# amathislab/BUCTD

Measured on AMD Instinct MI355X. Metric: images/sec (train) BUCTD-CoAM-W48 384x288, higher is better.
Workload: dtype f32 (3x3 convs: operands split exactly into 3 bf16 pieces, 6 bf16 MFMAs per product, fp32 accumulate - fp32-class); 1 GPU; BUCTD-CoAM-W48 (pose_hrnet_coam, ATT_MODULES [F,T,F,F], colored condition) 384x288 CrowdPose-14kpt full train step: fwd + JointsMSE + bwd + grad all-reduce + Adam + arg-max accuracy decode; global_batch=32, batch_per_gpu=32, input=N x 6 x 384 x 288 fp32, params=115581770, parallelism=dp1, hip_streams=4, conv_math=bf16x6, step_graph=False

## Files before the change

buctd_amd/_C.py:

```python
import ctypes as C
import os

import torch

_HERE = os.path.dirname(os.path.abspath(__file__))
LIB_PATH = os.path.join(_HERE, "lib", "libbuctd_hip.so")


class ConvDesc(C.Structure):
    _fields_ = [(n, C.c_int) for n in ("N", "H", "W", "Ci", "Co", "R", "S", "stride", "pad", "Ho", "Wo")]


class BasicBlockDesc(C.Structure):
    _fields_ = ([(n, C.c_int) for n in ("N", "H", "W", "C")] +
                [(n, C.c_void_p) for n in ("x", "w1_fwd", "w2_fwd", "w1_bwd", "w2_bwd", "gamma1", "beta1", "gamma2", "beta2",
                                           "running_mean1", "running_var1", "running_mean2", "running_var2")] +
                [(n, C.c_float) for n in ("eps1", "momentum1", "eps2", "momentum2")] +
                [(n, C.c_void_p) for n in ("z1", "z2", "y", "acc", "stat")])


class BasicBlockGrads(C.Structure):
    _fields_ = ([(n, C.c_void_p) for n in ("dy", "dz2", "dres", "dy1", "dz1", "dx", "dw1", "dw2", "dgamma1", "dbeta1",
                                           "dgamma2", "dbeta2")] +
                [(n, C.c_int) for n in ("acc_w1", "acc_w2", "acc_bn1", "acc_bn2")] +
# ... 208 lines not shown
    "buctd_gconv_x6_prep_item": (_I, [_I, _I, _I, _P, _I, _P, _P]),
    "buctd_gconv_x6_prep_batched": (_I, [_P, _I, _P]),
    "buctd_gconv_x6_stats_groups": (_I, [_I] * 6 + [_PI, _PI]),
    "buctd_gconv_x6_fwd": (_I, [_I] * 6 + [_P] * 6 + [_I, _P, _P, _P, _P]),
    "buctd_gconv_x6_dgrad": (_I, [_I] * 6 + [_P] * 4 + [_P]),
    "buctd_mha_fwd_bf16x6_workspace": (_SZ, [_I, _I, _I]),
    "buctd_mha_fwd_bf16x6_ws": (_I, [_I, _I, _I, _P, _P, _P, _I, _I, _F, _P, _P, _P, _SZ, _P]),
    "buctd_mha_train_supported": (_I, [_I, _I]),
    "buctd_mha_fwd_train": (_I, [_I, _I, _I, _P, _P, _P, _I, _I, _F, _F, _U64, _P, _P, _P]),
    "buctd_mha_bwd_workspace": (_SZ, [_I, _I]),
    "buctd_mha_bwd": (_I, [_I, _I, _I, _P, _P, _P, _I, _I, _P, _P, _P, _F, _F, _U64, _P, _P, _I, _P, _I, _P, _SZ, _P]),
    "buctd_mha_fwd_train_dseed": (_I, [_I, _I, _I, _P, _P, _P, _I, _I, _F, _F, _P, _P, _P, _P]),
    "buctd_mha_bwd_dseed": (_I, [_I, _I, _I, _P, _P, _P, _I, _I, _P, _P, _P, _F, _F, _P, _P, _P, _I, _P, _I, _P, _SZ, _P]),
    "buctd_mha_heads_fwd_supported": (_I, [_I, _I, _I]),
    "buctd_mha_heads_fwd": (_I, [C.POINTER(MhaArgs), _P]),
    "buctd_mha_heads_fwd_bf16x6": (_I, [C.POINTER(MhaArgs), _P]),
    "buctd_mha_heads_train_supported": (_I, [_I, _I, _I]),
    "buctd_mha_heads_fwd_train": (_I, [C.POINTER(MhaArgs), _U64, _P]),
    "buctd_mha_heads_bwd_workspace": (_SZ, [_I, _I, _I]),
    "buctd_mha_heads_bwd": (_I, [C.POINTER(MhaArgs), _U64, _P, _SZ, _P]),
    "buctd_mha_heads_fwd_train_dseed": (_I, [C.POINTER(MhaArgs), _P, _P]),
    "buctd_mha_heads_bwd_dseed": (_I, [C.POINTER(MhaArgs), _P, _P, _SZ, _P]),
    "buctd_nms_workspace": (_SZ, [_I]),
    "buctd_nms": (_I, [_P, _P, _P, _I, _I, _F, _P, _SZ, _P]),
    "buctd_cpu_nms": (_I, [_P, _I, _P, _F, _P, _P]),
    "buctd_argmax_decode_refined": (_I, [_P, _I, _I, _I, _P, _P, _P, _P, _P]),
    "buctd_argmax_decode_dark": (_I, [_P, _I, _I, _I, _P, _P, _P, _P, _P]),
    "buctd_gaussian_target": (_I, [_P, _P, _I, _I, _I, _I, _F, _F, _F, _P, _P, _P]),
    "buctd_cond_render_workspace": (_SZ, [_I, _I, _I, _I]),
    "buctd_cond_render": (_I, [_P, _I, _P, _I, _I, _I, _I, _I, _I, _P, _P, _SZ, _P]),
    "buctd_flipback_avg": (_I, [_P, _P, _P, _I, _I, _I, _I, _I, _P, _P]),
    "buctd_sgd_step": (_I, [_P, _P, _P, _L, _F, _F, _F, _I, _I, _F, _P]),
    "buctd_adam_step": (_I, [_P, _P, _P, _P, _L, _F, _F, _F, _F, _I, _F, _P]),
    "buctd_bf16_pack_conv": (_I, [_P, _L, _L, _L, _L, _I, _I, _I, _P, _P, _P, _P, _P, _F, _P, _P, _P]),
    "buctd_bf16_conv": (_I, [_P, _I, _I, _I, _I, _P, _P, _I, _I, _I, _I, _P, _I, _I, _P, _P, _SZ, _P]),
    "buctd_bf16_fuse_sum": (_I, [C.POINTER(_P), _PI, _I, _I, _I, _I, _I, _I, _P, _P]),
    "buctd_bf16_from_f32": (_I, [_P, _L, _P, _P]),
}

_lib = None


class BuctdHipError(RuntimeError):
    pass


def lib():
    global _lib
    if _lib is None:
        if not os.path.isfile(LIB_PATH):
            raise BuctdHipError(
                f"{LIB_PATH} is missing - build it with `make` (or __graft_entry__.build()); "
                "buctd_amd has no CPU / eager fallback")
        handle = C.CDLL(LIB_PATH, mode=C.RTLD_GLOBAL)
        for name, (res, args) in SIGNATURES.items():
            fn = getattr(handle, name)
            fn.restype = res
            fn.argtypes = args
        _lib = handle
    return _lib


def check(rc, what=""):
    if rc != 0:
        msg = lib().buctd_last_error()
        raise BuctdHipError(f"{what} failed ({rc}): {msg.decode() if msg else ''}")
# ... 23 lines not shown
```

buctd_amd/csrc/conv_gather_x6.hip:

```cpp
#include "c3_lean.h"
#include <string.h>

#define GC_MAXT 9
#define GC_TAB_OFF (56 * 1024)

struct GcClass {
  int ntaps, nhs, nsteps;
  int oy0, ox0;
  long wp_off;
  unsigned pdy, pdx;
};

struct GcArgs {
  C3Args e;
  const float* src;
  const unsigned char* wp;
  int SH, SWd, SC, ss, cpt;
  int ncls;
  GcClass cls[4];
};

template <int MF, int NF, int WM, int WN, int MODE>
__global__ __launch_bounds__(256, 2) void gconv_x6_kernel(GcArgs p) {
  constexpr int BM = WM * MF * 16, BN = WN * NF * 16, ROWB = 96, PST = 32, BROW = 192;
  constexpr int QA = BM / 64;
  static_assert(WM * WN == 4 && BM % 64 == 0, "four waves, BM a multiple of 64");
  extern __shared__ __attribute__((aligned(16))) unsigned char smem[];
  const int t = threadIdx.x, lane = t & 63, wave = t >> 6;
  const int i16 = lane & 15, g = lane >> 4;
  const int wave_m = wave % WM, wave_n = wave / WM;
  const int bx = blockIdx.x, by = blockIdx.y;
  const GcClass& c = p.cls[blockIdx.z];
  C3Args e = p.e;
  e.oy0 = c.oy0; e.ox0 = c.ox0;
  const int p0 = bx * BM, n0 = by * BN;

// ... 94 lines not shown
      }
#undef GC_MMA
      if (mf < 2 * QA && mf < MF) {
        const int h = mf / QA, q = mf % QA;
        split_store_pk<3, PST>(smem + (size_t)(1 - SET) * ABUF + ((size_t)h * BM + arow + RSTEP * q) * ROWB, c4 * 4,
                               areg[1 - SET][h][q]);
      }
      __builtin_amdgcn_sched_barrier(0);
    }
    if (2 * QA > MF) {
#pragma unroll
      for (int i = MF; i < 2 * QA; ++i) {
        const int h = i / QA, q = i % QA;
        split_store_pk<3, PST>(smem + (size_t)(1 - SET) * ABUF + ((size_t)h * BM + arow + RSTEP * q) * ROWB, c4 * 4,
                               areg[1 - SET][h][q]);
      }
    }
    if (!PRIV) __syncthreads();
  };

  load_a(0, areg[0]);
  load_b(0, bnx[0]);
  load_a(1, areg[1]);
  store_a(areg[0], 0);
  if (!PRIV) __syncthreads();
  for (int st = 0; st < c.nsteps; st += 2) {
    step(st, IC<0>{});
    if (st + 1 < c.nsteps) step(st + 1, IC<1>{});
  }
  __syncthreads();
  if constexpr (MODE < 0) c3_epilogue<MF, NF, WM, WN>(e, acc, smem, bx, by, p0, n0);
  else c3l_epilogue<MF, NF, WM, WN, MODE>(e, acc, smem, reinterpret_cast<float*>(smem + GC_TAB_OFF), p0, n0);
}

struct GcPrep {
  const float* w;
  unsigned char* out;
  int Co, Ci, R, S, dir;
  int ncls;
  int ntaps[4], nsteps[4];
  long off[4];
  int tr[4][GC_MAXT], ts[4][GC_MAXT];
  long items[4];
};

__device__ __forceinline__ void gc_prep_body(const GcPrep& p) {
  const int nrows = p.dir ? p.Ci : p.Co, kc = p.dir ? p.Co : p.Ci, cpt = kc / 16;
  const long total = p.items[p.ncls - 1];
  for (long idx = (long)blockIdx.x * 256 + threadIdx.x; idx < total; idx += (long)gridDim.x * 256) {
    int cl = 0;
    while (idx >= p.items[cl]) ++cl;
    const long li = idx - (cl ? p.items[cl - 1] : 0);
    const int ks = (int)(li & 31);
    const long sr = li >> 5;
    const int row = (int)(sr % nrows), st = (int)(sr / nrows);
    const int hs = 2 * st + (ks >> 4);
    float v = 0.f;
    if (hs < p.ntaps[cl] * cpt) {
      const int tp = hs / cpt, k = (hs - tp * cpt) * 16 + (ks & 15);
      const int r = p.tr[cl][tp], s = p.ts[cl][tp];
      const int co = p.dir ? k : row, ci = p.dir ? row : k;
      v = p.w[(((long)co * p.R + r) * p.S + s) * p.Ci + ci];
    }
    unsigned char* o = p.out + p.off[cl] + ((size_t)st * nrows + row) * 192 + ks * 2;
#pragma unroll
    for (int q = 0; q < 3; ++q) {
      const __bf16 h = (__bf16)v;
      *reinterpret_cast<unsigned short*>(o + q * 64) = __builtin_bit_cast(unsigned short, h);
      v -= (float)h;
    }
  }
}

__global__ __launch_bounds__(256) void gconv_x6_prep_kernel(GcPrep p) { gc_prep_body(p); }

__global__ __launch_bounds__(256) void gconv_x6_prep_batched_kernel(const GcPrep* __restrict__ items) {
  gc_prep_body(items[blockIdx.y]);
// ... 417 lines not shown
```

buctd_amd/csrc/loss_decode.hip:

```cpp
#include "common.h"
#include "../../include/buctd_hip.h"

__global__ __launch_bounds__(256) void mse_partial_kernel(const float* __restrict__ pred, const float* __restrict__ gt,
                                                          const float* __restrict__ w, int HW, float gcoef,
                                                          float* __restrict__ part, float* __restrict__ grad) {
  __shared__ float sm[4];
  const long row = blockIdx.x;
  const float wt = w ? w[row] : 1.f;
  const float w2 = wt * wt;
  float s = 0.f;
  for (int i = threadIdx.x; i < HW; i += 256) {
    const float d = pred[row * HW + i] - gt[row * HW + i];
    s += d * d;
    if (grad) grad[row * HW + i] = gcoef * w2 * d;
  }
  s = block_sum_256(s, sm);
  if (threadIdx.x == 0) part[row] = s * w2;
}
__global__ __launch_bounds__(256) void mse_final_kernel(const float* __restrict__ part, int n, float coef,
                                                        float* __restrict__ loss) {
  __shared__ float sm[4];
  double s = 0.0;
  for (int i = threadIdx.x; i < n; i += 256) s += (double)part[i];
  float f = block_sum_256((float)s, sm);
  if (threadIdx.x == 0) loss[0] = f * coef;
}
extern "C" int buctd_joints_mse(const float* pred, const float* gt, const float* w, int N, int K, int HW, float* loss,
                                float* grad, float gscale, void* workspace, size_t workspace_bytes, void* stream) {
  BUCTD_CHECK_ARG(pred && gt && loss && N > 0 && K > 0 && HW > 0, "buctd_joints_mse: bad argument");
  const size_t need = (size_t)N * K * sizeof(float);
  if (!workspace || workspace_bytes < need) {
    buctd_set_error("buctd_joints_mse: workspace %zu bytes < required %zu", workspace_bytes, need);
    return BUCTD_EWORKSPACE;
// ... 494 lines not shown

__global__ __launch_bounds__(256) void flipback_avg_kernel(const float* __restrict__ a, const float* __restrict__ b,
                                                           const int32_t* __restrict__ perm, int K, int H, int W,
                                                           int shift, long total, float* __restrict__ out) {
  const long step = (long)gridDim.x * 256;
  for (long i = (long)blockIdx.x * 256 + threadIdx.x; i < total; i += step) {
    const int x = (int)(i % W);
    long r = i / W;
    const int y = (int)(r % H);
    r /= H;
    const int k = (int)(r % K);
    const long n = r / K;
    const int xs = (shift && x >= 1) ? x - 1 : x;
    const float fv = b[((n * K + perm[k]) * H + y) * W + (W - 1 - xs)];
    out[i] = (a[i] + fv) * 0.5f;
  }
}
extern "C" int buctd_flipback_avg(const float* a, const float* b, const int32_t* perm, int N, int K, int H, int W,
                                  int shift, float* out, void* stream) {
  BUCTD_CHECK_ARG(a && b && perm && out && N > 0 && K > 0 && H > 0 && W > 0, "buctd_flipback_avg: bad argument");
  const long total = (long)N * K * H * W;
  long blocks = (total + 255) / 256;
  if (blocks > 4096) blocks = 4096;
  hipLaunchKernelGGL(flipback_avg_kernel, dim3((unsigned)blocks), dim3(256), 0, (hipStream_t)stream, a, b, perm, K, H,
                     W, shift, total, out);
  BUCTD_CHECK_LAUNCH("buctd_flipback_avg");
  return BUCTD_OK;
}

__global__ __launch_bounds__(256) void adam_kernel(float* __restrict__ p, const float* __restrict__ g,
                                                   float* __restrict__ m, float* __restrict__ v, long n, float lr,
                                                   float b1, float b2, float eps, float bc1, float bc2_sqrt,
                                                   float gscale) {
  const float step_size = lr / bc1;
  const long n4 = n >> 2;
  const long step = (long)gridDim.x * 256;
  for (long i = (long)blockIdx.x * 256 + threadIdx.x; i < n4; i += step) {
    f32x4 pp = reinterpret_cast<f32x4*>(p)[i];
    const f32x4 gg = reinterpret_cast<const f32x4*>(g)[i] * gscale;
    f32x4 mm = reinterpret_cast<f32x4*>(m)[i];
    f32x4 vv = reinterpret_cast<f32x4*>(v)[i];
#pragma unroll
    for (int j = 0; j < 4; ++j) {
      mm[j] = b1 * mm[j] + (1.f - b1) * gg[j];
      vv[j] = b2 * vv[j] + (1.f - b2) * gg[j] * gg[j];
      const float denom = sqrtf(vv[j]) / bc2_sqrt + eps;
      pp[j] -= step_size * (mm[j] / denom);
    }
    reinterpret_cast<f32x4*>(p)[i] = pp;
    reinterpret_cast<f32x4*>(m)[i] = mm;
    reinterpret_cast<f32x4*>(v)[i] = vv;
  }
  for (long i = n4 * 4 + (long)blockIdx.x * 256 + threadIdx.x; i < n; i += step) {
    const float gg = g[i] * gscale;
    const float mm = b1 * m[i] + (1.f - b1) * gg;
    const float vv = b2 * v[i] + (1.f - b2) * gg * gg;
    m[i] = mm;
    v[i] = vv;
    p[i] -= step_size * (mm / (sqrtf(vv) / bc2_sqrt + eps));
  }
}
extern "C" int buctd_adam_step(float* p, const float* g, float* m, float* v, long n, float lr, float beta1,
                               float beta2, float eps, int step, float gscale, void* stream) {
  BUCTD_CHECK_ARG(p && g && m && v && n > 0 && step >= 1, "buctd_adam_step: bad argument");
  const double bc1 = 1.0 - pow((double)beta1, (double)step);
  const double bc2 = 1.0 - pow((double)beta2, (double)step);
  long blocks = ((n + 3) / 4 + 255) / 256;
  if (blocks > 4096) blocks = 4096;
  hipLaunchKernelGGL(adam_kernel, dim3((unsigned)blocks), dim3(256), 0, (hipStream_t)stream, p, g, m, v, n, lr, beta1,
                     beta2, eps, (float)bc1, (float)sqrt(bc2), gscale);
  BUCTD_CHECK_LAUNCH("buctd_adam_step");
  return BUCTD_OK;
}

__global__ __launch_bounds__(256) void sgd_kernel(float* __restrict__ p, const float* __restrict__ g, float* __restrict__ buf,
                                                  long n, float lr, float mu, float wd, int nesterov, int first, float gscale) {
  const long step = (long)gridDim.x * 256;
  for (long i = (long)blockIdx.x * 256 + threadIdx.x; i < n; i += step) {
    float pp = p[i];
    float gg = g[i] * gscale + wd * pp;
    if (mu != 0.f) {
      const float b = first ? gg : mu * buf[i] + gg;
      buf[i] = b;
      gg = nesterov ? gg + mu * b : b;
    }
    p[i] = pp - lr * gg;
  }
}
extern "C" int buctd_sgd_step(float* p, const float* g, float* momentum_buf, long n, float lr, float momentum,
                              float weight_decay, int nesterov, int first_step, float gscale, void* stream) {
  BUCTD_CHECK_ARG(p && g && n > 0 && (momentum == 0.f || momentum_buf), "buctd_sgd_step: bad argument");
  long blocks = (n + 255) / 256;
// ... 7 lines not shown
```

buctd_amd/engine.py:

```python
import os
import time

import torch
import torch.distributed as dist

from . import nn as bnn
from . import ops

_ALIGN = 4


class FlatParams:

    def __init__(self, module):
        bnn.prepare_module(module)
        self.params = []
        seen = set()
        for p in module.parameters():
            if id(p) not in seen:
                seen.add(id(p))
                self.params.append(p)
        if not self.params:
            raise ValueError("module has no parameters")
        dev = self.params[0].device
        self.offsets = {}
        off = 0
        for p in self.params:
            if p.dtype != torch.float32 or p.device != dev:
                raise ValueError("all parameters must be fp32 on one device")
            self.offsets[id(p)] = off
            off += (p.numel() + _ALIGN - 1) // _ALIGN * _ALIGN
        self.numel = off
        self.flat = torch.zeros(off, dtype=torch.float32, device=dev)
        self.grad = torch.zeros(off, dtype=torch.float32, device=dev)
        self._gviews = {}
        for p in self.params:
            v = self._view(self.flat, p)
            v.copy_(p.data)
            p.data = v
            self._gviews[id(p)] = self._view(self.grad, p)
        self.ready_cb = None
        ops.set_grad_arena(self)

    def _view(self, buf, p):
        o = self.offsets[id(p)]
        return torch.as_strided(buf, p.shape, p.stride(), o)

    def span(self, p):
        o = self.offsets[id(p)]
        return o, o + p.numel()

    def __call__(self, p):
        return self._gviews.get(id(p))

    def owns(self, p):
        return id(p) in self._gviews

    def grad_is_arena(self, p):
        return p.grad is not None and p.grad.data_ptr() == self._gviews[id(p)].data_ptr()

    def collect(self):
        for p in self.params:
            g = self._gviews[id(p)]
            if p.grad is None:
                if p.requires_grad:
                    g.zero_()
            elif not self.grad_is_arena(p):
                g.copy_(p.grad)
                p.grad = g

    def grad_runs(self):
        runs = []
        for p in self.params:
            if p.grad is None:
                continue
            s = self.offsets[id(p)]
            e = s + (p.numel() + _ALIGN - 1) // _ALIGN * _ALIGN
            if runs and runs[-1][1] == s:
                runs[-1][1] = e
            else:
                runs.append([s, e])
        return [(s, e) for s, e in runs]


class FusedAdam(torch.optim.Optimizer):

    def __init__(self, flat, lr=1e-3, betas=(0.9, 0.999), eps=1e-8, grad_sync=None):
        if not isinstance(flat, FlatParams):
            raise TypeError("FusedAdam works on an engine.FlatParams arena")
        super().__init__(flat.params, dict(lr=lr, betas=betas, eps=eps))
        self.flat = flat
        self.exp_avg = torch.zeros_like(flat.flat)
        self.exp_avg_sq = torch.zeros_like(flat.flat)
        self.step_count = 0
        self.grad_sync = grad_sync

    @torch.no_grad()
    def step(self, closure=None):
        if closure is not None:
            raise NotImplementedError("closures are not used on the BUCTD path")
        self.flat.collect()
        gscale = self.grad_sync() if self.grad_sync is not None else 1.0
        self.step_count += 1
        g = self.param_groups[0]
        ops.adam_step(self.flat.flat, self.flat.grad, self.exp_avg, self.exp_avg_sq, g["lr"], g["betas"][0],
                      g["betas"][1], g["eps"], self.step_count, gscale)
        ops.weights_updated()
        ops.refresh_prepared(self.flat.flat.device)
        if self.flat.flat.is_cuda:
            ops.acc_pool.reset(self.flat.flat.device)

    def zero_grad(self, set_to_none=True):
        self.zeroed = getattr(self, "zeroed", 0) + 1
        for p in self.flat.params:
            p.grad = None

    def state_dict(self):
        state = {}
        if self.step_count > 0:
            for i, p in enumerate(self.flat.params):
                o, e = self.flat.span(p)
                state[i] = {"step": torch.tensor(float(self.step_count)),
                            "exp_avg": torch.as_strided(self.exp_avg, p.shape, p.stride(), o).clone(),
                            "exp_avg_sq": torch.as_strided(self.exp_avg_sq, p.shape, p.stride(), o).clone()}
        groups = []
        for g in self.param_groups:
            d = {k: v for k, v in g.items() if k != "params"}
            for k, v in (("weight_decay", 0), ("amsgrad", False), ("maximize", False)):
                d.setdefault(k, v)
            d["params"] = list(range(len(self.flat.params)))
            groups.append(d)
        return {"state": state, "param_groups": groups}

    def load_state_dict(self, sd):
        if "state" not in sd:
            self.step_count = int(sd["step"])
            self.exp_avg.copy_(sd["exp_avg"])
            self.exp_avg_sq.copy_(sd["exp_avg_sq"])
        else:
            state = sd["state"]
# ... 648 lines not shown
```

buctd_amd/ops.py:

```python
import ctypes as C
import math

import torch

from . import _C
from ._C import ConvDesc, MatmulDesc, check, lib, ptr, stream_ptr

_capture = {"on": False, "events": set(), "allow_seeds": False, "seed_table": None, "seed_draws": 0}
_SEED_TABLE_SLOTS = 1024


def capturing():
    return _capture["on"]


def _new_event(stream=None):
    ev = torch.cuda.Event()
    ev.record(stream) if stream is not None else ev.record()
    if _capture["on"]:
        _capture["events"].add(id(ev))
        _capture.setdefault("keep", []).append(ev)
    return ev


# ... 413 lines not shown
    if _conv_math["mode"] != "bf16x6":
        return False
    items, live = [], []
    for ref in _gprep_registry["weights"]:
        w = ref()
        if w is None or not w.is_cuda or w.device != device:
            continue
        cache = getattr(w, "_buctd_gprep", None)
        if cache is None or cache[0][0] != w.data_ptr():
            continue
        live.append(ref)
        if cache[0] == (w.data_ptr(), w._version, epoch):
            continue
        Co, Ci = _wshape(w)[0], _wshape(w)[1]
        for direction in (0, 1):
            img = cache[2 + direction]
            if img is not None:
                items.append((cache[1], Ci, Co, w.data_ptr(), direction, img.data_ptr()))
        cache[0] = (w.data_ptr(), w._version, epoch)
    _gprep_registry["weights"] = live
    if not items:
        return False
    key = tuple(items)
    if _gprep_registry["table_key"] != key:
        isz = int(lib().buctd_gconv_x6_prep_item_bytes())
        buf = C.create_string_buffer(isz * len(items))
        base = C.addressof(buf)
        for i, (kind, Ci, Co, wptr, direction, iptr) in enumerate(items):
            check(lib().buctd_gconv_x6_prep_item(kind, Ci, Co, C.c_void_p(wptr), direction, C.c_void_p(iptr),
                                                 C.c_void_p(base + i * isz)), "gconv_x6_prep_item")
        _gprep_registry["table"] = torch.frombuffer(bytearray(buf.raw), dtype=torch.uint8).to(device)
        _gprep_registry["table_key"] = key
    check(lib().buctd_gconv_x6_prep_batched(ptr(_gprep_registry["table"]), len(items), stream_ptr()), "gconv_x6_prep_batched")
    return True


def _conv3x3_prepared(w, flip):
    import weakref
    Co, Ci = _wshape(w)[0], _wshape(w)[1]
    epoch = _weights_epoch["n"]
    key = (w.data_ptr(), w._version, epoch, _conv_math["mode"])
    cache = getattr(w, "_buctd_prep", None)
    if cache is not None and cache[0] != key and cache[0][:2] == key[:2] and cache[0][3:] == key[3:]:
        _prep_all(w.device)
    if cache is None or cache[0] != key:
        first = cache is None
        cache = [key, None, None]
        try:
            w._buctd_prep = cache
            if first:
                _prep_registry["weights"].append(weakref.ref(w))
        except (AttributeError, RuntimeError, TypeError):
            pass
    if cache[1 + flip] is None:
        nbytes = _c3fn("_prep_bytes")(Ci, Co, flip)
        img = torch.empty(nbytes, dtype=torch.uint8, device=w.device)
        check(_c3fn("_prep")(Ci, Co, ptr(w), flip, ptr(img), stream_ptr()), "conv3x3 prep")
        cache[1 + flip] = img
    _prep_wait(w.device)
    return cache[1 + flip]


def _conv3x3_bf16x3(x, w, flip, cin, cout, bias, scale, shift, residual, relu, stats, in_bn=None):
    N, H, W = x.shape[0], x.shape[1], x.shape[2]
    wp = _conv3x3_prepared(w, flip)
    y = torch.empty((N, H, W, cout), dtype=torch.float32, device=x.device)
# ... 429 lines not shown
           Kc=None, gsa=0, gsbk=0, Nc=None, gsbn=0, gsc=0, alpha=1.0, bias=None, bias_axis=0,
           a_off=0, b_off=0, c_off=0):
    d = MatmulDesc(batch, M, N, K, a_layout, b_layout, lda, ldb, ldc, stride_a, stride_b, stride_c,
                   K if Kc is None else Kc, gsa, gsbk, N if Nc is None else Nc, gsbn, gsc, alpha, bias_axis)
    need = lib().buctd_matmul_workspace(C.byref(d))
    ws = workspace(need, A.device) if need else None
    pa = C.c_void_p(A.data_ptr() + 4 * a_off)
    pb = C.c_void_p(B.data_ptr() + 4 * b_off)
    pc = C.c_void_p(Cout.data_ptr() + 4 * c_off)
    check(lib().buctd_matmul(C.byref(d), pa, pb, ptr(bias), pc, ptr(ws), ws.numel() if ws is not None else 0,
                             stream_ptr()), "matmul")
    return Cout


def x6_image(src, V, K, role, *, vs, ks, vg=0, vgs=0, kg=0, kgs=0, off=0, out=None):
    need = lib().buctd_x6_image_bytes(V, K, role)
    if out is None or out.numel() < need:
        out = torch.empty(need, dtype=torch.uint8, device=src.device)
    check(lib().buctd_x6_image(C.c_void_p(src.data_ptr() + 4 * off), V, K, vg, vgs, vs, kg, kgs, ks, role, ptr(out),
                               stream_ptr()), "x6_image")
    return out


def x6_gemm(a_image, b_image, Cout, M, N, K, *, ldc, Nc=0, gsc=0, bias=None, bias_axis=0, alpha=1.0, c_off=0):
    check(lib().buctd_x6_gemm(M, N, K, ptr(a_image), ptr(b_image), ptr(bias), bias_axis, alpha,
                              C.c_void_p(Cout.data_ptr() + 4 * c_off), ldc, Nc, gsc, stream_ptr()), "x6_gemm")
    return Cout


def _x6_weight_image(w, V, K, transposed):
    key = (w.data_ptr(), w._version, _weights_epoch["n"])
    cache = getattr(w, "_buctd_x6img", None)
    if cache is None or cache["key"] != key:
        cache = {"key": key}
        try:
            w._buctd_x6img = cache
        except (AttributeError, RuntimeError, TypeError):
            pass
    tag = "t" if transposed else "n"
    if tag not in cache:
        ld = w.shape[1]
        cache[tag] = x6_image(w, V, K, 0, vs=1, ks=ld) if transposed else x6_image(w, V, K, 0, vs=ld, ks=1)
        cache[tag + "_ev"] = _new_event()
        cache[tag + "_stream"] = torch.cuda.current_stream(w.device).cuda_stream
    elif torch.cuda.current_stream(w.device).cuda_stream != cache[tag + "_stream"]:
        _wait_event(torch.cuda.current_stream(w.device), cache[tag + "_ev"])
    return cache[tag]


def fc_o_x6_ok(T, rows):
    return _conv_math["mode"] == "bf16x6" and T >= 512 and rows >= 192


def bn_finalize(part, info, rows, Cn, eps, momentum, running_mean, running_var):
    mean = torch.empty(Cn, dtype=torch.float32, device=part.device)
    invstd = torch.empty(Cn, dtype=torch.float32, device=part.device)
    counts = info[2] if len(info) > 2 else None
    check(lib().buctd_bn_finalize(ptr(part), ptr(counts), info[0], info[1], rows, Cn, eps, momentum, ptr(mean), ptr(invstd),
                                  ptr(running_mean), ptr(running_var), stream_ptr()), "bn_finalize")
    return mean, invstd


class BnAccInput:

    def __init__(self, acc, rows, bn, training=True, relu=True):
        Cn = acc.Cn
        dev = bn.weight.device
        self.acc, self.rows, self.gamma, self.beta, self.relu = acc, int(rows), bn.weight, bn.bias, relu
        self.eps = bn.eps
        self.momentum = 0.1 if bn.momentum is None else bn.momentum
        stat = torch.empty((2, Cn), dtype=torch.float32, device=dev)
        self.mean, self.invstd = stat[0], stat[1]
        track = bn.track_running_stats and training
        self.rm = bn.running_mean if track else None
        self.rv = bn.running_var if track else None
# ... 1369 lines not shown
```

include/buctd_hip.h:

```cpp
#ifndef BUCTD_HIP_H
#define BUCTD_HIP_H
#include <stddef.h>
#include <stdint.h>

#ifdef __cplusplus
extern "C" {
#endif

int buctd_version(void);
const char* buctd_last_error(void);

typedef struct {
  int N, H, W, Ci;
  int Co, R, S;
  int stride, pad;
  int Ho, Wo;
} buctd_conv_desc;

int buctd_conv2d_fwd_thin(const buctd_conv_desc* d);
int buctd_conv2d_fwd(const buctd_conv_desc* d, const float* x, const float* w, const float* bias,
                     const float* scale, const float* shift, const float* residual, int relu, float* y,
                     float* stats_partials, void* stream);
int buctd_conv2d_dgrad(const buctd_conv_desc* d, const float* dy, const float* w, const float* bias, float* dx,
                       float* stats_partials, void* stream);
// ... 277 lines not shown
  float eps1, momentum1, eps2, momentum2;
  float *z1, *z2, *y;
  void* acc;
  float* stat;
} buctd_basic_block;
typedef struct {
  const float* dy;
  float *dz2, *dres, *dy1, *dz1;
  float* dx;
  float *dw1, *dw2, *dgamma1, *dbeta1, *dgamma2, *dbeta2;
  int acc_w1, acc_w2, acc_bn1, acc_bn2;
  void* bn_acc;
  void* wg_ws; size_t wg_ws_bytes;
} buctd_basic_block_grads;
int buctd_basic_chain_fwd_train(int n, const buctd_basic_block* blocks, void* stream);
int buctd_basic_chain_bwd(int n, const buctd_basic_block* blocks, const buctd_basic_block_grads* grads, void* stream,
                          void* side_stream);

int buctd_basic_branches_fwd_train(int nb, int n, const buctd_basic_block* blocks, void* stream);
int buctd_basic_branches_bwd(int nb, int n, const buctd_basic_block* blocks, const buctd_basic_block_grads* grads, void* stream,
                             void* side_stream);

int buctd_stream_fork(void* from, void* to);

int buctd_x6_image_dims(int V, int K, int role, int* Vpad, int* Kpad);
size_t buctd_x6_image_bytes(int V, int K, int role);
int buctd_x6_image(const float* src, int V, int K, int vg, long vgs, long vs, int kg, long kgs, long ks, int role,
                   void* image, void* stream);
int buctd_x6_gemm(int M, int N, int K, const void* a_image, const void* b_image, const float* bias, int bias_axis,
                  float alpha, float* C, long ldc, int Nc, long gsc, void* stream);

int buctd_adam_step(float* p, const float* g, float* m, float* v, long n, float lr, float beta1, float beta2,
                    float eps, int step, float gscale, void* stream);
int buctd_sgd_step(float* p, const float* g, float* momentum_buf, long n, float lr, float momentum, float weight_decay,
                   int nesterov, int first_step, float gscale, void* stream);

int buctd_mha_fwd_supported(int T, int d);
int buctd_mha_fwd(int B, int T, int d, const float* q, const float* k, const float* v, int ldqk, int ldv, float scale,
                  float* out, float* lse, void* stream);
int buctd_mha_fwd_bf16x6(int B, int T, int d, const float* q, const float* k, const float* v, int ldqk, int ldv,
                         float scale, float* out, float* lse, void* stream);
size_t buctd_mha_fwd_bf16x6_workspace(int B, int T, int d);
int buctd_mha_fwd_bf16x6_ws(int B, int T, int d, const float* q, const float* k, const float* v, int ldqk, int ldv,
                            float scale, float* out, float* lse, void* workspace, size_t workspace_bytes, void* stream);
int buctd_mha_train_supported(int T, int d);
int buctd_mha_fwd_train(int B, int T, int d, const float* q, const float* k, const float* v, int ldqk, int ldv, float scale,
                        float p_drop, uint64_t seed, float* out, float* lse, void* stream);
size_t buctd_mha_bwd_workspace(int B, int T);
int buctd_mha_bwd(int B, int T, int d, const float* q, const float* k, const float* v, int ldqk, int ldv, const float* out,
                  const float* dout, const float* lse, float scale, float p_drop, uint64_t seed, float* dq, float* dk,
                  int lddqk, float* dv, int lddv, void* workspace, size_t workspace_bytes, void* stream);
int buctd_mha_fwd_train_dseed(int B, int T, int d, const float* q, const float* k, const float* v, int ldqk, int ldv,
                              float scale, float p_drop, const uint64_t* seed, float* out, float* lse, void* stream);
int buctd_mha_bwd_dseed(int B, int T, int d, const float* q, const float* k, const float* v, int ldqk, int ldv,
                        const float* out, const float* dout, const float* lse, float scale, float p_drop,
                        const uint64_t* seed, float* dq, float* dk, int lddqk, float* dv, int lddv, void* workspace,
                        size_t workspace_bytes, void* stream);

typedef struct buctd_mha_args {
  int B, T, h, dh;
  const float* q; const float* k; const float* v;
  int ldq, ldk, ldv;
  float* out; int ldo;
  float* lse;
  float scale, p_drop;
  const float* dout; int lddo;
// ... 129 lines not shown
```

Measured before the change: 516.5 images/s.

## Fuse Adam update with regeneration of bf16x6 split weight images

Adds a kernel that performs the Adam update tile by tile and, from the updated weights held in LDS, directly writes the 3-piece bf16 split images used by the 3x3, gathered, and FC x6 kernels. The host builds a unit/item table mapping flat parameter offsets to cached images and marks those caches as current, so the next step skips the separate per-weight repacking passes. This removes a full re-read of all ~115M parameters and many small prep launches, but adds table-building logic, cache-key bookkeeping, and scattered writes in the optimizer kernel.

```diff
diff --git a/buctd_amd/_C.py b/buctd_amd/_C.py
--- a/buctd_amd/_C.py
+++ b/buctd_amd/_C.py
@@ -264,6 +264,8 @@
     "buctd_flipback_avg": (_I, [_P, _P, _P, _I, _I, _I, _I, _I, _P, _P]),
     "buctd_sgd_step": (_I, [_P, _P, _P, _L, _F, _F, _F, _I, _I, _F, _P]),
     "buctd_adam_step": (_I, [_P, _P, _P, _P, _L, _F, _F, _F, _F, _I, _F, _P]),
+    "buctd_adam_step_images": (_I, [_P, _P, _P, _P, _F, _F, _F, _F, _I, _F, _P, _I, _P, _P, _P]),
+    "buctd_adam_step_images_geometry": (_I, [_PI, _PI, _PI, _PI, _PI, _PI, _PI]),
     "buctd_bf16_pack_conv": (_I, [_P, _L, _L, _L, _L, _I, _I, _I, _P, _P, _P, _P, _P, _F, _P, _P, _P]),
     "buctd_bf16_conv": (_I, [_P, _I, _I, _I, _I, _P, _P, _I, _I, _I, _I, _P, _I, _I, _P, _P, _SZ, _P]),
     "buctd_bf16_fuse_sum": (_I, [C.POINTER(_P), _PI, _I, _I, _I, _I, _I, _I, _P, _P]),
diff --git a/buctd_amd/csrc/adam_core.h b/buctd_amd/csrc/adam_core.h
--- /dev/null
+++ b/buctd_amd/csrc/adam_core.h
@@ -0,0 +1,39 @@
+#pragma once
+#include "common.h"
+
+struct AdamConst {
+  float b1, b2, eps, bc2_sqrt, step_size, gscale;
+};
+
+__device__ __forceinline__ AdamConst adam_const(float lr, float b1, float b2, float eps, float bc1, float bc2_sqrt,
+                                                float gscale) {
+  AdamConst c;
+  c.b1 = b1; c.b2 = b2; c.eps = eps; c.bc2_sqrt = bc2_sqrt; c.step_size = lr / bc1; c.gscale = gscale;
+  return c;
+}
+
+__device__ __forceinline__ void adam_update(float& p, float g, float& m, float& v, const AdamConst& c) {
+  const float gg = g * c.gscale;
+  m = c.b1 * m + (1.f - c.b1) * gg;
+  v = c.b2 * v + (1.f - c.b2) * gg * gg;
+  const float denom = sqrtf(v) / c.bc2_sqrt + c.eps;
+  p -= c.step_size * (m / denom);
+}
+
+__device__ __forceinline__ f32x4 adam_update4(float* __restrict__ p, const float* __restrict__ g, float* __restrict__ m,
+                                              float* __restrict__ v, long i, const AdamConst& c) {
+  f32x4 pp = reinterpret_cast<f32x4*>(p)[i];
+  const f32x4 gg = reinterpret_cast<const f32x4*>(g)[i];
+  f32x4 mm = reinterpret_cast<f32x4*>(m)[i];
+  f32x4 vv = reinterpret_cast<f32x4*>(v)[i];
+#pragma unroll
+  for (int j = 0; j < 4; ++j) {
+    float pj = pp[j], mj = mm[j], vj = vv[j];
+    adam_update(pj, gg[j], mj, vj, c);
+    pp[j] = pj; mm[j] = mj; vv[j] = vj;
+  }
+  reinterpret_cast<f32x4*>(p)[i] = pp;
+  reinterpret_cast<f32x4*>(m)[i] = mm;
+  reinterpret_cast<f32x4*>(v)[i] = vv;
+  return pp;
+}
diff --git a/buctd_amd/csrc/adam_images.hip b/buctd_amd/csrc/adam_images.hip
--- /dev/null
+++ b/buctd_amd/csrc/adam_images.hip
@@ -0,0 +1,192 @@
+#include "common.h"
+#include "adam_core.h"
+#include "gc_prep.h"
+#include "../../include/buctd_hip.h"
+
+typedef unsigned short ai_u16x8 __attribute__((ext_vector_type(8)));
+
+namespace {
+constexpr int AI_C3_CW = 32, AI_G1_CW = 256, AI_FC_R = 32, AI_FC_CW = 64;
+constexpr int AI_LDS_FLOATS = 144 * (AI_C3_CW + 4);
+static_assert(16 * (AI_G1_CW + 4) <= AI_LDS_FLOATS && AI_FC_R * (AI_FC_CW + 4) <= AI_LDS_FLOATS, "LDS tile");
+
+template <int PST>
+__device__ __forceinline__ void split8_store(unsigned char* o, const float (&x)[8]) {
+  ai_u16x8 h, m, l;
+#pragma unroll
+  for (int e = 0; e < 8; ++e) {
+    const __bf16 hh = (__bf16)x[e];
+    const float r1 = x[e] - (float)hh;
+    const __bf16 mm = (__bf16)r1;
+    const __bf16 ll = (__bf16)(r1 - (float)mm);
+    h[e] = __builtin_bit_cast(unsigned short, hh);
+    m[e] = __builtin_bit_cast(unsigned short, mm);
+    l[e] = __builtin_bit_cast(unsigned short, ll);
+  }
+  *reinterpret_cast<ai_u16x8*>(o) = h;
+  *reinterpret_cast<ai_u16x8*>(o + PST) = m;
+  *reinterpret_cast<ai_u16x8*>(o + 2 * PST) = l;
+}
+
+__device__ __forceinline__ void load8(float (&x)[8], const float* t) {
+  const f32x4 a = *reinterpret_cast<const f32x4*>(t);
+  const f32x4 b = *reinterpret_cast<const f32x4*>(t + 4);
+  x[0] = a.x; x[1] = a.y; x[2] = a.z; x[3] = a.w; x[4] = b.x; x[5] = b.y; x[6] = b.z; x[7] = b.w;
+}
+
+__device__ __forceinline__ void emit_c3(const buctd_adam_item& it, const buctd_adam_unit& u, const float* tile, int cw, int LS) {
+  const int nh = cw >> 4, ntask = nh * 5 * 64;
+  unsigned char* fwd = reinterpret_cast<unsigned char*>(it.img[0]);
+  unsigned char* flp = reinterpret_cast<unsigned char*>(it.img[1]);
+  for (int k = threadIdx.x; k < ntask; k += 256) {
+    const int lane = k & 63, hs = k >> 6;
+    const int h = hs / 5, s = hs - h * 5;
+    const int g4 = lane >> 4, nl = lane & 15;
+    const int tap = 2 * s + (g4 >> 1);
+    float x[8];
+    if (fwd) {
+#pragma unroll
+      for (int e = 0; e < 8; ++e) x[e] = 0.f;
+      if (tap < 9) load8(x, tile + (nl * 9 + tap) * LS + h * 16 + (g4 & 1) * 8);
+      const size_t step = (size_t)((u.t1 >> 4) + h) * 5 + s;
+      split8_store<1024>(fwd + (step * (it.rows >> 4) + (u.t0 >> 4)) * 3072 + lane * 16, x);
+    }
+    if (flp) {
+#pragma unroll
+      for (int e = 0; e < 8; ++e) x[e] = tap < 9 ? tile[(((g4 & 1) * 8 + e) * 9 + (8 - tap)) * LS + h * 16 + nl] : 0.f;
+      const size_t step = (size_t)(u.t0 >> 4) * 5 + s;
+      split8_store<1024>(flp + (step * (it.cols >> 4) + (u.t1 >> 4) + h) * 3072 + lane * 16, x);
+    }
+  }
+}
+
+__device__ __forceinline__ void emit_gc(const buctd_adam_item& it, const buctd_adam_unit& u, const GcPrep* __restrict__ gcs,
+                                        const float* tile, int cw, int LS) {
+  const int ntap = it.ntap;
+  if (it.gc[0] >= 0) {
+    const GcPrep* G = gcs + it.gc[0];
+    const int cpt = it.cols >> 4, nt = G->ntaps[0];
+    const int ntask = (cw >> 4) * nt * 32;
+    for (int k = threadIdx.x; k < ntask; k += 256) {
+      const int e = k & 1, row = (k >> 1) & 15, rest = k >> 5;
+      const int h = rest / nt, tp = rest - h * nt;
+      const int ti = G->tr[0][tp] * G->S + G->ts[0][tp];
+      const int hs = tp * cpt + (u.t1 >> 4) + h;
+      float x[8];
+      load8(x, tile + (row * ntap + ti) * LS + h * 16 + e * 8);
+      split8_store<64>(G->out + G->off[0] + ((size_t)(hs >> 1) * it.rows + u.t0 + row) * 192 + (hs & 1) * 32 + e * 16, x);
+    }
+  }
+  if (it.gc[1] >= 0) {
+    const GcPrep* G = gcs + it.gc[1];
+    const int cpt = it.rows >> 4;
+    int ntall = 0;
+    for (int c = 0; c < G->ncls; ++c) ntall += G->ntaps[c];
+    const int ntask = ntall * cw * 2;
+    for (int k = threadIdx.x; k < ntask; k += 256) {
+      const int e = k & 1, r2 = k >> 1;
+      int tp = r2 / cw;
+      const int cil = r2 - tp * cw;
+      int cl = 0;
+      while (tp >= G->ntaps[cl]) { tp -= G->ntaps[cl]; ++cl; }
+      const int ti = G->tr[cl][tp] * G->S + G->ts[cl][tp];
+      const int hs = tp * cpt + (u.t0 >> 4);
+      float x[8];
+#pragma unroll
+      for (int j = 0; j < 8; ++j) x[j] = tile[((e * 8 + j) * ntap + ti) * LS + cil];
+      split8_store<64>(G->out + G->off[cl] + ((size_t)(hs >> 1) * it.cols + u.t1 + cil) * 192 + (hs & 1) * 32 + e * 16, x);
+    }
+  }
+}
+
+__device__ __forceinline__ void emit_fc(const buctd_adam_item& it, const buctd_adam_unit& u, const float* tile, int LS) {
+  const int k = threadIdx.x, lane = k & 63, blk = k >> 6;
+  float x[8];
+  if (it.img[0]) {
+    const int rl = (blk & 1) * 16 + (lane & 15), cl0 = (blk >> 1) * 32 + (lane >> 4) * 8;
+    const int v = u.t0 + rl, k0 = u.t1 + cl0;
+    if (v < it.rows && k0 < it.cols) {
+#pragma unroll
+      for (int e = 0; e < 8; ++e) x[e] = k0 + e < it.cols ? tile[rl * LS + cl0 + e] : 0.f;
+      const size_t kbn = (size_t)((it.cols + 255) >> 8) * 8;
+      split8_store<1024>(reinterpret_cast<unsigned char*>(it.img[0]) + ((size_t)(v >> 4) * kbn + (k0 >> 5)) * 3072 + lane * 16, x);
+    }
+  }
+  if (it.img[1]) {
+    const int vl = blk * 16 + (lane & 15), rl0 = (lane >> 4) * 8;
+    const int v = u.t1 + vl, k0 = u.t0 + rl0;
+    if (v < it.cols && k0 < it.rows) {
+#pragma unroll
+      for (int e = 0; e < 8; ++e) x[e] = k0 + e < it.rows ? tile[(rl0 + e) * LS + vl] : 0.f;
+      const size_t kbn = (size_t)((it.rows + 255) >> 8) * 8;
+      split8_store<1024>(reinterpret_cast<unsigned char*>(it.img[1]) + ((size_t)(v >> 4) * kbn + (k0 >> 5)) * 3072 + lane * 16, x);
+    }
+  }
+}
+
+__global__ __launch_bounds__(256) void adam_images_kernel(float* __restrict__ p, const float* __restrict__ g,
+                                                          float* __restrict__ m, float* __restrict__ v,
+                                                          const buctd_adam_unit* __restrict__ units,
+                                                          const buctd_adam_item* __restrict__ items,
+                                                          const GcPrep* __restrict__ gcs, float lr, float b1, float b2,
+                                                          float eps, float bc1, float bc2_sqrt, float gscale) {
+  __shared__ __attribute__((aligned(16))) float tile[AI_LDS_FLOATS];
+  const AdamConst c = adam_const(lr, b1, b2, eps, bc1, bc2_sqrt, gscale);
+  const buctd_adam_unit u = units[blockIdx.x];
+  const int t = threadIdx.x;
+  if (u.item < 0) {
+    const long q0 = u.off >> 2;
+    const int n4 = u.n >> 2;
+    for (int i = t; i < n4; i += 256) adam_update4(p, g, m, v, q0 + i, c);
+    return;
+  }
+  const buctd_adam_item it = items[u.item];
+  int nrow, cw, LS;
+  long base;
+  if (it.kind == 3) {
+    nrow = min(AI_FC_R, it.rows - u.t0);
+    cw = min(AI_FC_CW, it.cols - u.t1);
+    LS = AI_FC_CW + 4;
+    base = u.off + (long)u.t0 * it.cols + u.t1;
+  } else {
+    const int cmax = it.ntap == 1 ? AI_G1_CW : AI_C3_CW;
+    nrow = 16 * it.ntap;
+    cw = min(cmax, it.cols - u.t1);
+    LS = cmax + 4;
+    base = u.off + (long)u.t0 * it.ntap * it.cols + u.t1;
+  }
+  const int qpr = cw >> 2, nq = nrow * qpr;
+  for (int q = t; q < nq; q += 256) {
+    const int r = q / qpr, c4 = q - r * qpr;
+    const f32x4 pp = adam_update4(p, g, m, v, (base + (long)r * it.cols) / 4 + c4, c);
+    *reinterpret_cast<f32x4*>(tile + r * LS + c4 * 4) = pp;
+  }
+  __syncthreads();
+  if (it.kind == 1) emit_c3(it, u, tile, cw, LS);
+  else if (it.kind == 2) emit_gc(it, u, gcs, tile, cw, LS);
+  else emit_fc(it, u, tile, LS);
+}
+}
+
+extern "C" int buctd_adam_step_images(float* p, const float* g, float* m, float* v, float lr, float beta1, float beta2,
+                                      float eps, int step, float gscale, const buctd_adam_unit* units_device, int nunits,
+                                      const buctd_adam_item* items_device, const void* gathered_items_device, void* stream) {
+  BUCTD_CHECK_ARG(p && g && m && v && step >= 1 && units_device && nunits > 0 && items_device,
+                  "buctd_adam_step_images: bad argument");
+  const double bc1 = 1.0 - pow((double)beta1, (double)step);
+  const double bc2 = 1.0 - pow((double)beta2, (double)step);
+  hipLaunchKernelGGL(adam_images_kernel, dim3((unsigned)nunits), dim3(256), 0, (hipStream_t)stream, p, g, m, v, units_device,
+                     items_device, (const GcPrep*)gathered_items_device, lr, beta1, beta2, eps, (float)bc1, (float)sqrt(bc2),
+                     gscale);
+  BUCTD_CHECK_LAUNCH("buctd_adam_step_images");
+  return BUCTD_OK;
+}
+
+extern "C" int buctd_adam_step_images_geometry(int* unit_bytes, int* item_bytes, int* flat_run, int* c3_cols, int* g1_cols,
+                                               int* fc_rows, int* fc_cols) {
+  BUCTD_CHECK_ARG(unit_bytes && item_bytes && flat_run && c3_cols && g1_cols && fc_rows && fc_cols,
+                  "buctd_adam_step_images_geometry: null pointer");
+  *unit_bytes = (int)sizeof(buctd_adam_unit); *item_bytes = (int)sizeof(buctd_adam_item);
+  *flat_run = 8192; *c3_cols = AI_C3_CW; *g1_cols = AI_G1_CW; *fc_rows = AI_FC_R; *fc_cols = AI_FC_CW;
+  return BUCTD_OK;
+}
diff --git a/buctd_amd/csrc/conv_gather_x6.hip b/buctd_amd/csrc/conv_gather_x6.hip
--- a/buctd_amd/csrc/conv_gather_x6.hip
+++ b/buctd_amd/csrc/conv_gather_x6.hip
@@ -1,7 +1,7 @@
 #include "c3_lean.h"
+#include "gc_prep.h"
 #include <string.h>
 
-#define GC_MAXT 9
 #define GC_TAB_OFF (56 * 1024)
 
 struct GcClass {
@@ -162,17 +162,6 @@
   if constexpr (MODE < 0) c3_epilogue<MF, NF, WM, WN>(e, acc, smem, bx, by, p0, n0);
   else c3l_epilogue<MF, NF, WM, WN, MODE>(e, acc, smem, reinterpret_cast<float*>(smem + GC_TAB_OFF), p0, n0);
 }
-
-struct GcPrep {
-  const float* w;
-  unsigned char* out;
-  int Co, Ci, R, S, dir;
-  int ncls;
-  int ntaps[4], nsteps[4];
-  long off[4];
-  int tr[4][GC_MAXT], ts[4][GC_MAXT];
-  long items[4];
-};
 
 __device__ __forceinline__ void gc_prep_body(const GcPrep& p) {
   const int nrows = p.dir ? p.Ci : p.Co, kc = p.dir ? p.Co : p.Ci, cpt = kc / 16;
diff --git a/buctd_amd/csrc/gc_prep.h b/buctd_amd/csrc/gc_prep.h
--- /dev/null
+++ b/buctd_amd/csrc/gc_prep.h
@@ -0,0 +1,14 @@
+#pragma once
+
+#define GC_MAXT 9
+
+struct GcPrep {
+  const float* w;
+  unsigned char* out;
+  int Co, Ci, R, S, dir;
+  int ncls;
+  int ntaps[4], nsteps[4];
+  long off[4];
+  int tr[4][GC_MAXT], ts[4][GC_MAXT];
+  long items[4];
+};
diff --git a/buctd_amd/csrc/loss_decode.hip b/buctd_amd/csrc/loss_decode.hip
--- a/buctd_amd/csrc/loss_decode.hip
+++ b/buctd_amd/csrc/loss_decode.hip
@@ -1,4 +1,5 @@
 #include "common.h"
+#include "adam_core.h"
 #include "../../include/buctd_hip.h"
 
 __global__ __launch_bounds__(256) void mse_partial_kernel(const float* __restrict__ pred, const float* __restrict__ gt,
@@ -559,32 +560,16 @@
                                                    float* __restrict__ m, float* __restrict__ v, long n, float lr,
                                                    float b1, float b2, float eps, float bc1, float bc2_sqrt,
                                                    float gscale) {
-  const float step_size = lr / bc1;
+  const AdamConst c = adam_const(lr, b1, b2, eps, bc1, bc2_sqrt, gscale);
   const long n4 = n >> 2;
   const long step = (long)gridDim.x * 256;
-  for (long i = (long)blockIdx.x * 256 + threadIdx.x; i < n4; i += step) {
-    f32x4 pp = reinterpret_cast<f32x4*>(p)[i];
-    const f32x4 gg = reinterpret_cast<const f32x4*>(g)[i] * gscale;
-    f32x4 mm = reinterpret_cast<f32x4*>(m)[i];
-    f32x4 vv = reinterpret_cast<f32x4*>(v)[i];
-#pragma unroll
-    for (int j = 0; j < 4; ++j) {
-      mm[j] = b1 * mm[j] + (1.f - b1) * gg[j];
-      vv[j] = b2 * vv[j] + (1.f - b2) * gg[j] * gg[j];
-      const float denom = sqrtf(vv[j]) / bc2_sqrt + eps;
-      pp[j] -= step_size * (mm[j] / denom);
-    }
-    reinterpret_cast<f32x4*>(p)[i] = pp;
-    reinterpret_cast<f32x4*>(m)[i] = mm;
-    reinterpret_cast<f32x4*>(v)[i] = vv;
-  }
+  for (long i = (long)blockIdx.x * 256 + threadIdx.x; i < n4; i += step) adam_update4(p, g, m, v, i, c);
   for (long i = n4 * 4 + (long)blockIdx.x * 256 + threadIdx.x; i < n; i += step) {
-    const float gg = g[i] * gscale;
-    const float mm = b1 * m[i] + (1.f - b1) * gg;
-    const float vv = b2 * v[i] + (1.f - b2) * gg * gg;
+    float pp = p[i], mm = m[i], vv = v[i];
+    adam_update(pp, g[i], mm, vv, c);
     m[i] = mm;
     v[i] = vv;
-    p[i] -= step_size * (mm / (sqrtf(vv) / bc2_sqrt + eps));
+    p[i] = pp;
   }
 }
 extern "C" int buctd_adam_step(float* p, const float* g, float* m, float* v, long n, float lr, float beta1,
diff --git a/buctd_amd/engine.py b/buctd_amd/engine.py
--- a/buctd_amd/engine.py
+++ b/buctd_amd/engine.py
@@ -40,6 +40,7 @@
             p.data = v
             self._gviews[id(p)] = self._view(self.grad, p)
         self.ready_cb = None
+        self._ptr_index = None
         ops.set_grad_arena(self)
 
     def _view(self, buf, p):
@@ -49,6 +50,12 @@
     def span(self, p):
         o = self.offsets[id(p)]
         return o, o + p.numel()
+
+    def ptr_index(self):
+        if self._ptr_index is None:
+            base = self.flat.data_ptr()
+            self._ptr_index = {base + 4 * self.offsets[id(p)]: p for p in self.params if p.numel() > 0}
+        return self._ptr_index
 
     def __call__(self, p):
         return self._gviews.get(id(p))
@@ -94,6 +101,7 @@
         self.exp_avg_sq = torch.zeros_like(flat.flat)
         self.step_count = 0
         self.grad_sync = grad_sync
+        self.fuse_images = True
 
     @torch.no_grad()
     def step(self, closure=None):
@@ -103,9 +111,11 @@
         gscale = self.grad_sync() if self.grad_sync is not None else 1.0
         self.step_count += 1
         g = self.param_groups[0]
-        ops.adam_step(self.flat.flat, self.flat.grad, self.exp_avg, self.exp_avg_sq, g["lr"], g["betas"][0],
-                      g["betas"][1], g["eps"], self.step_count, gscale)
-        ops.weights_updated()
+        if not (self.fuse_images and ops.adam_step_images(self.flat, self.exp_avg, self.exp_avg_sq, g["lr"], g["betas"][0],
+                                                          g["betas"][1], g["eps"], self.step_count, gscale)):
+            ops.adam_step(self.flat.flat, self.flat.grad, self.exp_avg, self.exp_avg_sq, g["lr"], g["betas"][0],
+                          g["betas"][1], g["eps"], self.step_count, gscale)
+            ops.weights_updated()
         ops.refresh_prepared(self.flat.flat.device)
         if self.flat.flat.is_cuda:
             ops.acc_pool.reset(self.flat.flat.device)
diff --git a/buctd_amd/ops.py b/buctd_amd/ops.py
--- a/buctd_amd/ops.py
+++ b/buctd_amd/ops.py
@@ -469,6 +469,177 @@
         _gprep_registry["table"] = torch.frombuffer(bytearray(buf.raw), dtype=torch.uint8).to(device)
         _gprep_registry["table_key"] = key
     check(lib().buctd_gconv_x6_prep_batched(ptr(_gprep_registry["table"]), len(items), stream_ptr()), "gconv_x6_prep_batched")
+    return True
+
+
+_adam_img = {"key": None, "units": None, "items": None, "gcs": None, "nunits": 0, "geometry": None}
+_x6_registry = {"weights": []}
+
+
+def _adam_img_geometry():
+    if _adam_img["geometry"] is None:
+        v = [C.c_int() for _ in range(7)]
+        check(lib().buctd_adam_step_images_geometry(*[C.byref(x) for x in v]), "adam_step_images_geometry")
+        _adam_img["geometry"] = tuple(x.value for x in v)
+    return _adam_img["geometry"]
+
+
+def adam_image_units(runs, items, geometry):
+    import numpy as np
+    _, _, flat_run, c3_cols, g1_cols, fc_rows, fc_cols = geometry
+    dt = np.dtype([("off", "<i8"), ("n", "<i4"), ("item", "<i4"), ("t0", "<i4"), ("t1", "<i4")])
+    parts = []
+
+    def flat(s, e):
+        if e > s:
+            u = np.zeros((e - s + flat_run - 1) // flat_run, dt)
+            u["off"] = s + flat_run * np.arange(len(u), dtype=np.int64)
+            u["n"] = np.minimum(flat_run, e - u["off"])
+            u["item"] = -1
+            parts.append(u)
+
+    i = 0
+    for s, e in runs:
+        pos = s
+        while i < len(items) and items[i][0] < e:
+            off, kind, rows, cols, ntap = items[i]
+            if off < pos or off + rows * cols * ntap > e:
+                raise _C.BuctdHipError("adam_image_units: a filter with images is not inside one gradient run")
+            flat(pos, off)
+            th, tw = (fc_rows, fc_cols) if kind == 3 else (16, g1_cols if ntap == 1 else c3_cols)
+            t0, t1 = np.meshgrid(np.arange(0, rows, th, dtype=np.int32), np.arange(0, cols, tw, dtype=np.int32), indexing="ij")
+            u = np.zeros(t0.size, dt)
+            u["off"], u["item"], u["t0"], u["t1"] = off, i, t0.ravel(), t1.ravel()
+            parts.append(u)
+            pos = off + rows * cols * ntap
+            i += 1
+        flat(pos, e)
+    if i != len(items):
+        raise _C.BuctdHipError("adam_image_units: a filter with images lies outside the gradient runs")
+    return np.concatenate(parts) if parts else np.zeros(0, dt)
+
+
+def _adam_image_items(flat, device, mode):
+    index = flat.ptr_index()
+    found = {}
+
+    def slot(w, numel):
+        p = index.get(w.data_ptr())
+        if p is None or p.grad is None or p.numel() != numel or w.numel() != numel or not w.is_cuda or w.device != device:
+            return None
+        off = flat.offsets[id(p)]
+        return None if off in found else off
+
+    for ref in _prep_registry["weights"]:
+        w = ref()
+        cache = getattr(w, "_buctd_prep", None) if w is not None else None
+        if cache is None or cache[0][0] != w.data_ptr() or cache[0][3] != mode or (cache[1] is None and cache[2] is None):
+            continue
+        Co, Ci = _wshape(w)[0], _wshape(w)[1]
+        off = slot(w, Co * Ci * 9)
+        if off is None or Ci % 16 or Co % 16 or any(
+                img is not None and img.numel() != lib().buctd_conv3x3_bf16x6_prep_bytes(Ci, Co, f)
+                for f, img in enumerate(cache[1:3])):
+            continue
+        found[off] = [1, Co, Ci, 9, cache[1], cache[2], cache, w]
+    for ref in _gprep_registry["weights"]:
+        w = ref()
+        cache = getattr(w, "_buctd_gprep", None) if w is not None else None
+        if cache is None or cache[0][0] != w.data_ptr() or cache[1] not in (1, 2) or (cache[2] is None and cache[3] is None):
+            continue
+        Co, Ci = _wshape(w)[0], _wshape(w)[1]
+        ntap = 1 if cache[1] == 1 else 9
+        off = slot(w, Co * Ci * ntap)
+        if off is None or Ci % 16 or Co % 16 or any(
+                img is not None and img.numel() != lib().buctd_gconv_x6_prep_bytes(cache[1], Ci, Co, d)
+                for d, img in enumerate(cache[2:4])):
+            continue
+        found[off] = [2, Co, Ci, ntap, cache[2], cache[3], cache, w]
+    live = []
+    for ref in _x6_registry["weights"]:
+        w = ref()
+        if w is None:
+            continue
+        live.append(ref)
+        cache = getattr(w, "_buctd_x6img", None)
+        if cache is None or cache["key"][0] != w.data_ptr() or w.dim() != 2 or not w.is_contiguous():
+            continue
+        rows, cols = w.shape
+        imgs = [cache.get(tag) if cache.get(tag + "_vk") == vk else None for tag, vk in (("n", (rows, cols)), ("t", (cols, rows)))]
+        off = slot(w, rows * cols)
+        if off is None or cols % 4 or (imgs[0] is None and imgs[1] is None) or any(
+                img is not None and img.numel() != lib().buctd_x6_image_bytes(V, K, 0)
+                for img, (V, K) in zip(imgs, ((rows, cols), (cols, rows)))):
+            continue
+        if any(tag in cache and img is None for tag, img in zip("nt", imgs)):
+            continue
+        found[off] = [3, rows, cols, 1, imgs[0], imgs[1], cache, w]
+    _x6_registry["weights"] = live
+    return found
+
+
+def adam_step_images(flat, m, v, lr, beta1, beta2, eps, step, gscale=1.0):
+    import numpy as np
+    mode = _conv_math["mode"]
+    if mode != "bf16x6" or not flat.flat.is_cuda:
+        return False
+    device = flat.flat.device
+    found = _adam_image_items(flat, device, mode)
+    if not found:
+        return False
+    runs = ((0, flat.numel),)
+    order = sorted(found)
+    key = (flat.flat.data_ptr(), flat.grad.data_ptr(), runs,
+           tuple((off,) + tuple(found[off][:4]) + tuple(None if t is None else t.data_ptr() for t in found[off][4:6])
+                 for off in order))
+    if _adam_img["key"] != key:
+        geometry = _adam_img_geometry()
+        gsz = int(lib().buctd_gconv_x6_prep_item_bytes())
+        idt = np.dtype([("kind", "<i4"), ("rows", "<i4"), ("cols", "<i4"), ("ntap", "<i4"), ("img", "<u8", 2), ("gc", "<i4", 2)])
+        if geometry[0] != 24 or geometry[1] != idt.itemsize:
+            raise _C.BuctdHipError("adam_step_images: table layouts of the library and of ops.py differ")
+        items = np.zeros(len(order), idt)
+        gbufs = []
+        for i, off in enumerate(order):
+            kind, rows, cols, ntap, img0, img1, cache, w = found[off]
+            items[i]["kind"], items[i]["rows"], items[i]["cols"], items[i]["ntap"] = kind, rows, cols, ntap
+            items[i]["gc"] = (-1, -1)
+            for d, img in enumerate((img0, img1)):
+                if img is None:
+                    continue
+                if kind != 2:
+                    items[i]["img"][d] = img.data_ptr()
+                    continue
+                buf = C.create_string_buffer(gsz)
+                check(lib().buctd_gconv_x6_prep_item(cache[1], cols, rows, ptr(w), d, ptr(img), buf), "gconv_x6_prep_item")
+                items[i]["gc"][d] = len(gbufs)
+                gbufs.append(buf.raw)
+        units = adam_image_units(runs, [(off,) + tuple(found[off][:4]) for off in order], geometry)
+
+        def up(raw):
+            return torch.frombuffer(bytearray(raw), dtype=torch.uint8).to(device)
+        _adam_img.update(key=key, units=up(units.tobytes()), items=up(items.tobytes()),
+                         gcs=up(b"".join(gbufs)) if gbufs else None, nunits=len(units))
+    check(lib().buctd_adam_step_images(ptr(flat.flat), ptr(flat.grad), ptr(m), ptr(v), lr, beta1, beta2, eps, step, gscale,
+                                       ptr(_adam_img["units"]), _adam_img["nunits"], ptr(_adam_img["items"]),
+                                       ptr(_adam_img["gcs"]), stream_ptr()), "adam_step_images")
+    weights_updated()
+    epoch = _weights_epoch["n"]
+    ev = torch.cuda.Event()
+    ev.record()
+    cur = torch.cuda.current_stream(device).cuda_stream
+    for kind, _, _, _, img0, img1, cache, w in found.values():
+        if kind == 1:
+            cache[0] = (w.data_ptr(), w._version, epoch, mode)
+        elif kind == 2:
+            cache[0] = (w.data_ptr(), w._version, epoch)
+        else:
+            cache["key"] = (w.data_ptr(), w._version, epoch)
+            for tag, img in (("n", img0), ("t", img1)):
+                if img is not None:
+                    cache[tag + "_ev"], cache[tag + "_stream"] = ev, cur
+    _prep_registry["event"], _prep_registry["stream"] = ev, cur
+    _prep_registry["waited"] = set()
     return True
 
 
@@ -964,15 +1135,20 @@
     key = (w.data_ptr(), w._version, _weights_epoch["n"])
     cache = getattr(w, "_buctd_x6img", None)
     if cache is None or cache["key"] != key:
+        first = cache is None
         cache = {"key": key}
         try:
             w._buctd_x6img = cache
+            if first:
+                import weakref
+                _x6_registry["weights"].append(weakref.ref(w))
         except (AttributeError, RuntimeError, TypeError):
             pass
     tag = "t" if transposed else "n"
     if tag not in cache:
         ld = w.shape[1]
         cache[tag] = x6_image(w, V, K, 0, vs=1, ks=ld) if transposed else x6_image(w, V, K, 0, vs=ld, ks=1)
+        cache[tag + "_vk"] = (V, K)
         cache[tag + "_ev"] = _new_event()
         cache[tag + "_stream"] = torch.cuda.current_stream(w.device).cuda_stream
     elif torch.cuda.current_stream(w.device).cuda_stream != cache[tag + "_stream"]:
diff --git a/include/buctd_hip.h b/include/buctd_hip.h
--- a/include/buctd_hip.h
+++ b/include/buctd_hip.h
@@ -333,6 +333,20 @@
 
 int buctd_adam_step(float* p, const float* g, float* m, float* v, long n, float lr, float beta1, float beta2,
                     float eps, int step, float gscale, void* stream);
+typedef struct {
+  long off;
+  int n, item, t0, t1;
+} buctd_adam_unit;
+typedef struct {
+  int kind, rows, cols, ntap;
+  void* img[2];
+  int gc[2];
+} buctd_adam_item;
+int buctd_adam_step_images(float* p, const float* g, float* m, float* v, float lr, float beta1, float beta2, float eps,
+                           int step, float gscale, const buctd_adam_unit* units_device, int nunits,
+                           const buctd_adam_item* items_device, const void* gathered_items_device, void* stream);
+int buctd_adam_step_images_geometry(int* unit_bytes, int* item_bytes, int* flat_run, int* c3_cols, int* g1_cols,
+                                    int* fc_rows, int* fc_cols);
 int buctd_sgd_step(float* p, const float* g, float* momentum_buf, long n, float lr, float momentum, float weight_decay,
                    int nesterov, int first_step, float gscale, void* stream);
 
```

Measured after the change: 520.6 images/s, median of 6. Within noise of the previous version (+0.8%).
